# glwagner/OldOceananigans.jl

Hardware: AMD Instinct MI355X
Metric: cell_updates_per_s (higher is better)
Workload: dtype f64

## Files before the change

### oldoceananigans.jl_amd/csrc/ocn_advect_split.h

```cpp
#pragma once
#include "ocn_kernels.h"
#include "ocn_tendency_roles.h"

__global__ void __launch_bounds__(256) sum_parent_kernel(const double *__restrict__ a, const double *__restrict__ b, double *__restrict__ out, long n) {
    const long stride = (long)gridDim.x * blockDim.x;
    for (long q = (long)blockIdx.x * blockDim.x + threadIdx.x; q < n; q += stride) out[q] = a[q] + b[q];
}

template <int F, bool ACC>
__global__ void __launch_bounds__(256) advective_tendency_kernel(DGrid g, FView ua, FView va, FView wa, FView psi, FView G, Range6 r) {
    const int i = r.i0 + blockIdx.x * blockDim.x + threadIdx.x;
    const int j = r.j0 + blockIdx.y * blockDim.y + threadIdx.y;
    const int k = r.k0 + blockIdx.z;
    if (i > r.i1 || j > r.j1 || k > r.k1) return;
    double dx, dy, dz, vinv;
    if (F == F_U) {
        vinv = g.vinv_c[k - 1 + g.Hz];
        dx = mom_flux<AQ_U, 0, true, 0, true>(g, ua, psi, i, j, k) - mom_flux<AQ_U, 0, true, 0, true>(g, ua, psi, i - 1, j, k);
        dy = mom_flux<AQ_V, 0, false, 1, false>(g, va, psi, i, j + 1, k) - mom_flux<AQ_V, 0, false, 1, false>(g, va, psi, i, j, k);
        dz = mom_flux<AQ_W, 0, false, 2, false>(g, wa, psi, i, j, k + 1) - mom_flux<AQ_W, 0, false, 2, false>(g, wa, psi, i, j, k);
    } else if (F == F_V) {
        vinv = g.vinv_c[k - 1 + g.Hz];
        dx = mom_flux<AQ_U, 1, false, 0, false>(g, ua, psi, i + 1, j, k) - mom_flux<AQ_U, 1, false, 0, false>(g, ua, psi, i, j, k);
        dy = mom_flux<AQ_V, 1, true, 1, true>(g, va, psi, i, j, k) - mom_flux<AQ_V, 1, true, 1, true>(g, va, psi, i, j - 1, k);
        dz = mom_flux<AQ_W, 1, false, 2, false>(g, wa, psi, i, j, k + 1) - mom_flux<AQ_W, 1, false, 2, false>(g, wa, psi, i, j, k);
    } else if (F == F_W) {
        vinv = g.vinv_f[k - 1 + g.Hz];
        dx = mom_flux<AQ_U, 2, false, 0, false>(g, ua, psi, i + 1, j, k) - mom_flux<AQ_U, 2, false, 0, false>(g, ua, psi, i, j, k);
        dy = mom_flux<AQ_V, 2, false, 1, false>(g, va, psi, i, j + 1, k) - mom_flux<AQ_V, 2, false, 1, false>(g, va, psi, i, j, k);
        dz = mom_flux<AQ_W, 2, true, 2, true>(g, wa, psi, i, j, k) - mom_flux<AQ_W, 2, true, 2, true>(g, wa, psi, i, j, k - 1);
    } else {
        vinv = g.vinv_c[k - 1 + g.Hz];
        dx = tracer_flux<0>(g, ua, psi, i + 1, j, k) - tracer_flux<0>(g, ua, psi, i, j, k);
        dy = tracer_flux<1>(g, va, psi, i, j + 1, k) - tracer_flux<1>(g, va, psi, i, j, k);
        dz = tracer_flux<2>(g, wa, psi, i, j, k + 1) - tracer_flux<2>(g, wa, psi, i, j, k);
    }
    const double div = vinv * ((dx + dy) + dz);
    if (ACC) G.at(i, j, k) = G.at(i, j, k) - div;
    else     G.at(i, j, k) = -div + 0.0;
}

struct RoleSplitArgs : RoleArgs<OCN_MAX_FIELDS> {
    const double *A[3];
    int nrole;
    int role[OCN_MAX_FIELDS];
};

template <int TY, bool BZ, bool ACC>
__global__ void __launch_bounds__(64 * (TY + 1), OCN_ROLE_WAVES) role_split_kernel(DGrid gin, RoleSplitArgs a) {
    __shared__ double FX[2][TY][66];
    __shared__ double FY[2][TY + 1][64];

    DGrid g = gin;
    g.tx = 0; g.ty = 0; g.tz = BZ ? 1 : 0;

    const unsigned d = blockIdx.x, xcd = d & 7u, slot = d >> 3, nr = (unsigned)a.nrole;
    const unsigned pair = xcd * (unsigned)a.band + slot / nr;
    if (slot / nr >= (unsigned)a.band || pair >= (unsigned)a.npair) return;
    const int fidx = a.role[slot % nr];
    const unsigned tile = pair % (unsigned)a.ntile, chunk = pair / (unsigned)a.ntile;
    const int i0 = a.r.i0 + (int)(tile % (unsigned)a.ntile_x) * 64, j0 = a.r.j0 + (int)(tile / (unsigned)a.ntile_x) * TY;
    const int kc0 = a.r.k0 + (int)chunk * a.kchunk;
    const int kc1 = min(kc0 + a.kchunk - 1, a.r.k1);
    if (fidx == 0) role_march<ROLE_U, TY, false, BZ, 0, false, RoleSplitArgs, true, ACC>(g, a, 0, i0, j0, kc0, kc1, FX, FY);
    else if (fidx == 1) role_march<ROLE_V, TY, false, BZ, 0, false, RoleSplitArgs, true, ACC>(g, a, 1, i0, j0, kc0, kc1, FX, FY);
    else if (fidx == 2) role_march<ROLE_W, TY, false, BZ, 0, false, RoleSplitArgs, true, ACC>(g, a, 2, i0, j0, kc0, kc1, FX, FY);
    else role_march<ROLE_C, TY, false, BZ, 0, false, RoleSplitArgs, true, ACC>(g, a, fidx, i0, j0, kc0, kc1, FX, FY);
}

static inline int launch_role_split(const OcnOptions &o, const DGrid &g, hipStream_t stream, const double *const adv[3], const double *const *psi,
                                    double *const *G, const int *roles, int nrole, const int *range, bool accumulate) {
    if (nrole <= 0) return 0;
    if (nrole > OCN_MAX_FIELDS || o.arithmetic != 0) return -2;
    RoleSplitArgs a;
    for (int f = 0; f < OCN_MAX_FIELDS; ++f) { a.U[f] = nullptr; a.G[f] = nullptr; a.Un[f] = nullptr; a.Gm[f] = nullptr; a.role[f] = 0; }
    a.ftab = nullptr;
    for (int c = 0; c < 3; ++c) a.A[c] = adv[c];
    a.nrole = nrole;
    for (int q = 0; q < nrole; ++q) {
        const int f = roles[q];
        if (f < 0 || f >= OCN_MAX_FIELDS || !psi[f] || !G[f]) return -2;
        a.role[q] = f; a.U[f] = psi[f]; a.G[f] = G[f];
    }
    a.has_zeta = 0; a.store_G = 1; a.dt = 0.0; a.gamma = 0.0; a.zeta = 0.0;
    const int Px = g.Nx + 2 * g.Hx, Py = g.Ny + 2 * g.Hy;
    a.s1 = Px;
    a.s2 = (unsigned)((long)Px * Py);
    a.off = (g.Hx - 1) + (long)Px * (g.Hy - 1);
    if (range) {
        a.r = Range6{range[0], range[1], range[2], range[3], range[4], range[5]};
        a.wk0 = a.r.k0;
    } else {
        a.r = Range6{1, g.Nx, 1, g.Ny, 1, g.Nz};
        a.wk0 = (g.tz != 0 && g.Nz > 1) ? 2 : 1;
    }
    constexpr int TY = OCN_ROLE_TY;
    const int nx = a.r.i1 - a.r.i0 + 1, ny = a.r.j1 - a.r.j0 + 1, nz = a.r.k1 - a.r.k0 + 1;
    if (nx <= 0 || ny <= 0 || nz <= 0) return 0;
    a.ntile_x = (nx + 63) / 64;
    a.ntile = a.ntile_x * ((ny + TY - 1) / TY);
    a.kchunk = o.role_kchunk > 0 ? o.role_kchunk : pick_role_kchunk((long)a.ntile * nrole, nz);
    const int nchunk = (nz + a.kchunk - 1) / a.kchunk;
    a.npair = a.ntile * nchunk;
    a.band = (a.npair + 7) / 8;
    const unsigned nblocks = (unsigned)a.band * 8u * (unsigned)nrole;
    const dim3 blk(64 * (TY + 1));
#define OCN_LAUNCH_SPLIT(BZV, ACCV) hipLaunchKernelGGL((role_split_kernel<TY, BZV, ACCV>), dim3(nblocks), blk, (size_t)o.role_ldspad, stream, g, a)
    if (g.tz != 0) { if (accumulate) OCN_LAUNCH_SPLIT(true, true); else OCN_LAUNCH_SPLIT(true, false); }
    else           { if (accumulate) OCN_LAUNCH_SPLIT(false, true); else OCN_LAUNCH_SPLIT(false, false); }
#undef OCN_LAUNCH_SPLIT
    return 0;
}
```

### oldoceananigans.jl_amd/csrc/ocn_api.hip

```cpp
#include "../../include/ocn_mi355x.h"
#include "ocn_kernels.h"
#include "ocn_options.h"
#include "ocn_tendency_fused.h"
#include "ocn_tendency_roles.h"
#include "ocn_advect_split.h"
#include "ocn_epilogue_march.h"
#include "ocn_forcing.h"
#include "ocn_implicit_z.h"
#include "ocn_particles.h"
#include "ocn_open_boundary.h"
#include "ocn_diagnostics.h"
#include "ocn_boundary_function.h"
#include "ocn_forcing_function.h"
#include <hipfft/hipfft.h>
#include <array>
#include <cfloat>
#include <cmath>
#include <cstdarg>
#include <cstdio>
#include <cstdlib>
#include <cstring>
#include <memory>
#include <string>
#include <utility>
// ... 1930 lines not shown
        *slot = total ? &m->tot[f] : const_cast<double **>(&m->bg[f]);
        *loc = m->loc[f];
        return OCN_OK;
    }
    if (q[0] == 'G' || q[0] == 'M') { kind = q[0]; ++q; }
    const int f = field_index(m, q);
    if (f < 0) return fail(OCN_EINVAL, "name %s not found in model.velocities or model.tracers.", name);
    *slot = kind == 'U' ? &m->U[f] : (kind == 'G' ? &m->Gn[f] : &m->Gm[f]);
    *loc = m->loc[f];
    return OCN_OK;
}

extern "C" int ocn_model_field(ocn_model_t m, const char *name, double **ptr, int loc[3]) {
    if (!m || !name || !ptr) return fail(OCN_EINVAL, "NULL argument");
    double **slot;
    int *l;
    int rc = field_lookup(m, name, &slot, &l);
    if (rc) return rc;
    *ptr = *slot;
    if (loc) memcpy(loc, l, sizeof(int) * 3);
    return OCN_OK;
}

enum OptionScope {
    OPT_STEP,
    OPT_CREATION,
    OPT_PARTITIONED,
};
struct OptionRow {
    const char *key;
    int OcnOptions::*member;
    OptionScope scope;
    bool (*valid)(int);
    const char *range;
    const char *alias;
};
static bool nonneg(int v) { return v >= 0; }
static bool onoff(int v) { return v == 0 || v == 1; }
static constexpr int kRoleStaticLds = 8 * (2 * OCN_ROLE_TY * 66 + 2 * (OCN_ROLE_TY + 1) * 64);
static constexpr int kRoleLdspadMax = 160 * 1024 - kRoleStaticLds;
static_assert(kRoleLdspadMax == 148256 || OCN_ROLE_TY != 7, "the message of role_ldspad states the bound at TY = 7");
static bool ldspad_fits(int v) { return v >= 0 && v <= kRoleLdspadMax; }
static const OptionRow kOptions[] = {
    {"tendency_impl", &OcnOptions::tendency_impl, OPT_STEP, [](int v) { return v >= 0 && v <= 2; }, "tendency_impl is 0, 1 or 2"},
    {"arithmetic", &OcnOptions::arithmetic, OPT_STEP, [](int v) { return v == 0 || v == 1; }, "arithmetic is 0 (reference sequence) or 1 (contracted)"},
    {"role_kchunk", &OcnOptions::role_kchunk, OPT_STEP, nonneg, "role_kchunk must be >= 0 (0 = automatic)"},
    {"role_ldspad", &OcnOptions::role_ldspad, OPT_STEP, ldspad_fits, "role_ldspad is 0 .. 148256 bytes (the 160 KiB of a CU minus the kernel's own LDS)"},
    {"fused_ty", &OcnOptions::fused_ty, OPT_STEP, [](int v) { return v == 3 || v == 7; }, "fused_ty is 3 or 7"},
    {"fused_kchunk", &OcnOptions::fused_kchunk, OPT_STEP, nonneg, "fused_kchunk must be >= 0 (0 = automatic)"},
    {"fused_zwin", &OcnOptions::fused_zwin, OPT_STEP, onoff, "fused_zwin is 0 or 1"},
    {"fused_xcd", &OcnOptions::fused_xcd, OPT_STEP, onoff, "fused_xcd is 0 or 1"},
    {"epilogue_march", &OcnOptions::epilogue_march, OPT_STEP, onoff, "epilogue_march is 0 or 1"},
    {"epilogue_rows", &OcnOptions::epilogue_rows, OPT_STEP, [](int v) { return v >= 1 && v <= 8; }, "epilogue_rows is 1 .. 8"},
    {"epilogue_kchunk", &OcnOptions::epilogue_kchunk, OPT_STEP, nonneg, "epilogue_kchunk must be >= 0 (0 = automatic)"},
    {"amd_march", &OcnOptions::amd_march, OPT_STEP, onoff, "amd_march is 0 or 1"},
    {"smag_march", &OcnOptions::smag_march, OPT_STEP, onoff, "smag_march is 0 or 1"},
    {"fused_halo", &OcnOptions::fused_halo, OPT_STEP, onoff, "fused_halo is 0 or 1"},
    {"real_fft", &OcnOptions::real_fft, OPT_STEP, onoff, "real_fft is 0 or 1"},
    {"c2r_strided", &OcnOptions::c2r_strided, OPT_CREATION, onoff, "c2r_strided is 0 or 1"},
    {"fused_zfft", &OcnOptions::fused_zfft, OPT_CREATION, onoff, "fused_zfft is 0 or 1"},
    {"split_solve", &OcnOptions::split_solve, OPT_STEP, onoff, "split_solve is 0 or 1"},
    {"line_zl512", &OcnOptions::line_zl512, OPT_STEP, [](int v) { return v == 4 || v == 8; }, "line_zl512 is 4 or 8"},
    {"skip_stage_pressure", &OcnOptions::skip_stage_pressure, OPT_STEP, onoff, "skip_stage_pressure is 0 or 1"},
    {"skip_dead_tendency_store", &OcnOptions::skip_dead_tendency_store, OPT_STEP, onoff, "skip_dead_tendency_store is 0 or 1"},
    {"dist_substructured", &OcnOptions::dist_substructured, OPT_CREATION, onoff, "dist_substructured is 0 or 1"},
    {"dist_zfirst", &OcnOptions::dist_zfirst, OPT_CREATION, onoff, "dist_zfirst is 0 or 1"},
    {"dist_xfast", &OcnOptions::dist_xfast, OPT_CREATION, onoff, "dist_xfast is 0 or 1"},
    {"dist_yline", &OcnOptions::dist_yline, OPT_CREATION, onoff, "dist_yline is 0 or 1"},
    {"dist_fuse_source", &OcnOptions::dist_fuse_source, OPT_STEP, onoff, "dist_fuse_source is 0 or 1"},
    {"dist_xline_group", &OcnOptions::dist_xline_group, OPT_STEP, onoff, "dist_xline_group is 0 or 1"},
    {"dist_pencil_transposes", &OcnOptions::dist_pencil_transposes, OPT_CREATION, onoff, "dist_pencil_transposes is 0 or 1"},
    {"swap_tendencies", &OcnOptions::swap_tendencies, OPT_STEP, onoff, "swap_tendencies is 0 or 1"},
    {"fuse_substep", &OcnOptions::fuse_substep, OPT_STEP, onoff, "fuse_substep is 0 or 1"},
    {"fused_epilogue", &OcnOptions::fused_epilogue, OPT_STEP, onoff, "fused_epilogue is 0 or 1"},
    {"fused_forcing", &OcnOptions::fused_forcing, OPT_STEP, onoff, "fused_forcing is 0 or 1"},
    {"use_graph", &OcnOptions::use_graph, OPT_STEP, onoff, "use_graph is 0 or 1"},
    {"async_halos", &OcnOptions::async_halos, OPT_PARTITIONED, [](int v) { return v >= -1 && v <= 1; }, "async_halos is -1 (automatic), 0 or 1"},
    {"thin_halos", &OcnOptions::thin_halos, OPT_PARTITIONED, onoff, "thin_halos is 0 or 1"},
    {"early_exchange", &OcnOptions::early_exchange, OPT_PARTITIONED, onoff, "early_exchange is 0 or 1"},
    {"strip_width", &OcnOptions::strip_width, OPT_PARTITIONED, nonneg, "strip_width must be >= 0 (0 = automatic)"},
    {"fused_step", &OcnOptions::fused_step, OPT_PARTITIONED, onoff, "fused_step is 0 or 1", "dist_fused_step"},
};

static const OptionRow *find_option(const char *key) {
    for (const OptionRow &r : kOptions)
        if (!strcmp(key, r.key) || (r.alias && !strcmp(key, r.alias))) return &r;
    return nullptr;
}
static const OptionRow *option_row(const char *key, int value) {
    const OptionRow *r = find_option(key);
    if (!r) { fail(OCN_EINVAL, "unknown option %s", key); return nullptr; }
    if (r->valid && !r->valid(value)) { fail(OCN_EINVAL, "%s", r->range); return nullptr; }
    return r;
}

extern "C" int ocn_set_option(const char *key, int value) {
    if (!key) return fail(OCN_EINVAL, "NULL argument");
    const OptionRow *r = option_row(key, value);
    if (!r) return OCN_EINVAL;
    g_defaults.*r->member = value;
    return OCN_OK;
}

static bool dist_fused_step_buffers(const ocn_model_s *m);
static int dist_model_get_option(const ocn_model_s *m, const char *key, int *value);
static void dist_abandon_exchange(ocn_model_s *m);
extern "C" int ocn_model_set_option(ocn_model_t m, const char *key, int value) {
    if (!m || !key) return fail(OCN_EINVAL, "NULL argument");
    m->epoch += 1;
    if (!strcmp(key, "profile")) { m->profile = value; m->events_used = 0; return OCN_OK; }
    if (!strcmp(key, "forcing_function_hoist")) {
        if (value != 0 && value != 1) return fail(OCN_EINVAL, "forcing_function_hoist is 0 or 1");
        m->ff.hoist = value != 0;
        return OCN_OK;
    }
    const OptionRow *r = option_row(key, value);
    if (!r) return OCN_EINVAL;
    if (r->scope == OPT_CREATION)
        return fail(OCN_ESTATE, "option %s is read when a model is created: set it with ocn_set_option before creating the model", key);
    if (r->scope == OPT_PARTITIONED && !m->dm) return fail(OCN_EINVAL, "option %s belongs to a partitioned model", key);
    if (r->member == &OcnOptions::fused_step && value && !dist_fused_step_buffers(m))
        return fail(OCN_ENOTSUP, "fused_step needs a (connected, Periodic, Periodic) slab with the z-fastest substructured solver");
    m->opt.*r->member = value;
    return OCN_OK;
}

static int model_ivd_form(const ocn_model_s *) { return 0; }

static int count_background(const ocn_model_s *m) {
    int n = 0;
    for (int f = 0; f < m->nf; ++f) n += m->bg[f] ? 1 : 0;
    return n;
}
static bool has_background(const ocn_model_s *m) { return count_background(m) > 0; }
static bool has_background_velocity(const ocn_model_s *m) { return m->bg[0] || m->bg[1] || m->bg[2]; }
static const double *total_velocity(const ocn_model_s *m, int c) { return m->bg[c] ? m->tot[c] : m->U[c]; }
static int update_total_velocities(ocn_model_s *m) {
    for (int c = 0; c < 3; ++c)
        if (m->bg[c]) {
            int rc = sum_parent(m->grid->d, m->U[c], m->bg[c], m->loc[c], m->tot[c]);
            if (rc) return rc;
        }
    return OCN_OK;
}

static bool has_forcing(const ocn_model_s *m) {
    for (int f = 0; f < m->nf; ++f)
        if (m->forcing_h.nterms[f] > 0) return true;
    return false;
}
static int evaluate_boundary_functions(ocn_model_s *m) {
    if (m->bf.n == 0) return OCN_OK;
    BfFields fields = {};
    for (int f = 0; f < m->nf; ++f) fields.p[f] = m->U[f];
    int na = 1, nb = 1;
    for (int q = 0; q < m->bf.n; ++q) { na = std::max(na, m->bf.slot[q].fn.Na); nb = std::max(nb, m->bf.slot[q].fn.Nb); }
    bf_launch(m->bf.table_d, m->bf.n, na, nb, fields, m->time);
    KERNEL_CHECK();
    return OCN_OK;
}

static int count_linear_flux(const ocn_model_s *m) {
    int n = 0;
    for (int f = 0; f < m->nf; ++f)
        for (int sd = 0; sd < 6; ++sd) n += m->lin[f][sd].on ? 1 : 0;
    return n;
}

struct StepPlan {
// ... 1565 lines not shown
```

### oldoceananigans.jl_amd/csrc/ocn_options.h

```cpp
#pragma once

struct OcnOptions {
    int tendency_impl = 2;
    int arithmetic = 0;
    int role_kchunk = 0;
    int role_ldspad = 0;
    int fused_ty = 7;
    int fused_kchunk = 0;
    int fused_zwin = 1;
    int fused_xcd = 0;
    int epilogue_march = 1;
    int epilogue_rows = 4;
    int epilogue_kchunk = 0;
    int amd_march = 1;
    int smag_march = 1;
    int fused_halo = 1;
    int real_fft = 1;
    int c2r_strided = 1;
    int fused_zfft = 1;
    int split_solve = 1;
    int line_zl512 = 4;
    int skip_stage_pressure = 1;
    int skip_dead_tendency_store = 1;
    int dist_substructured = 1;
    int dist_zfirst = 1;
    int dist_xfast = 1;
    int dist_yline = 1;
    int dist_fuse_source = 1;
    int dist_xline_group = 1;
    int dist_pencil_transposes = 1;
    int swap_tendencies = 1;
    int fuse_substep = 1;
    int fused_epilogue = 1;
    int fused_forcing = 1;
    int use_graph = 0;
    int async_halos = -1;
    int thin_halos = 1;
    int early_exchange = 1;
    int strip_width = 0;
    int fused_step = 1;
};
```

### oldoceananigans.jl_amd/csrc/ocn_tendency_roles.h

```cpp
#pragma once
#include "ocn_tendency_fused.h"
#include "ocn_forcing.h"

#ifndef OCN_ROLE_WAVES
#define OCN_ROLE_WAVES 6
#endif
#ifndef OCN_ROLE_TY
#define OCN_ROLE_TY 7
#endif
#ifndef OCN_ROLE_PF
#define OCN_ROLE_PF 1
#endif
#ifndef OCN_ROLE_ABLATE
#define OCN_ROLE_ABLATE 0
#endif
#ifndef OCN_ROLE_STORE_AUX
#define OCN_ROLE_STORE_AUX 2
#endif
#ifndef OCN_ROLE_GM_AUX
#define OCN_ROLE_GM_AUX 0
#endif
enum { ROLE_U = 0, ROLE_V = 1, ROLE_W = 2, ROLE_C = 3 };

template <int NF>
struct RoleArgs {
    const double *U[NF];
    double *G[NF];
    double *Un[NF];
    const double *Gm[NF];
    int s1;
    unsigned s2;
    long off;
    Range6 r;
    int wk0;
    int kchunk, ntile_x, ntile, npair, band;
    int has_zeta;
    int store_G;
    double dt, gamma, zeta;
    const ForcingTable *ftab;
};

typedef __amdgpu_buffer_rsrc_t Rsrc;
typedef unsigned v2u __attribute__((ext_vector_type(2)));
typedef const double __attribute__((address_space(4))) *KTab;
__device__ __forceinline__ KTab ktab(const double *p) { return (KTab)p; }
#define ROLE_OOB 0x80000000u
__device__ __forceinline__ Rsrc make_rsrc(const void *p) {
    return __builtin_amdgcn_make_buffer_rsrc(const_cast<void *>(p), 0, (int)ROLE_OOB, 0x00020000);
}
template <int IMM> __device__ __forceinline__ double ldb(Rsrc r, unsigned voff, unsigned soff) {
    return __builtin_bit_cast(double, __builtin_amdgcn_raw_buffer_load_b64(r, (int)(voff + (unsigned)IMM), (int)soff, 0));
}
template <int IMM> __device__ __forceinline__ double ldb_once(Rsrc r, unsigned voff, unsigned soff) {
    return __builtin_bit_cast(double, __builtin_amdgcn_raw_buffer_load_b64(r, (int)(voff + (unsigned)IMM), (int)soff, OCN_ROLE_GM_AUX));
}
template <int IMM> __device__ __forceinline__ void stb(Rsrc r, unsigned voff, unsigned soff, double v) {
    __builtin_amdgcn_raw_buffer_store_b64(__builtin_bit_cast(v2u, v), r, (int)(voff + (unsigned)IMM), (int)soff, OCN_ROLE_STORE_AUX);
}

struct ColOff { unsigned c; unsigned s1; };

template <bool OWN> __device__ __forceinline__ Win6 xwin6(Rsrc b, unsigned so, const ColOff &o, double centre) {
    Win6 w;
    w.s[0] = ldb<0>(b, o.c, so); w.s[1] = ldb<8>(b, o.c, so); w.s[2] = ldb<16>(b, o.c, so);
    w.s[3] = OWN ? centre : ldb<24>(b, o.c, so);
    w.s[4] = ldb<32>(b, o.c, so); w.s[5] = ldb<40>(b, o.c, so);
    return w;
}
__device__ __forceinline__ Win6 xwin4(Rsrc b, unsigned so, const ColOff &o) {
    Win6 w;
    w.s[0] = 0.0; w.s[5] = 0.0;
    w.s[1] = ldb<8>(b, o.c, so); w.s[2] = ldb<16>(b, o.c, so); w.s[3] = ldb<24>(b, o.c, so); w.s[4] = ldb<32>(b, o.c, so);
    return w;
}
template <bool OWN> __device__ __forceinline__ Win6 ywin6(Rsrc b, unsigned so, const ColOff &o, double centre) {
    Win6 w;
#pragma unroll
    for (int n = 0; n < 6; ++n) w.s[n] = (OWN && n == 3) ? centre : ldb<24>(b, o.c, so + (unsigned)(n - 3) * o.s1);
    return w;
}
__device__ __forceinline__ Win6 ywin4(Rsrc b, unsigned so, const ColOff &o) {
    Win6 w;
    w.s[0] = 0.0; w.s[5] = 0.0;
#pragma unroll
    for (int n = 1; n < 5; ++n) w.s[n] = ldb<24>(b, o.c, so + (unsigned)(n - 3) * o.s1);
    return w;
}
__device__ __forceinline__ Win6 zwin4(Rsrc b, unsigned so, const ColOff &o, unsigned s2) {
    Win6 w;
    w.s[0] = 0.0; w.s[5] = 0.0;
    w.s[1] = ldb<24>(b, o.c, so - 2u * s2); w.s[2] = ldb<24>(b, o.c, so - s2); w.s[3] = ldb<24>(b, o.c, so); w.s[4] = ldb<24>(b, o.c, so + s2);
    return w;
}

struct PlaneCtx {
    Rsrc u, v, w, q;
    unsigned so;
    unsigned s2;
    double axk, ayk;
    const double *axz, *ayz;
};

template <int ROLE, bool SPLIT = false> __device__ __forceinline__ Win6 load_zin(const PlaneCtx &p, unsigned so, const ColOff &o) {
    if (SPLIT && ROLE == ROLE_W) return zwin4(p.w, so, o, p.s2);
    if (ROLE == ROLE_U) return xwin4(p.w, so, o);
    if (ROLE == ROLE_V) return ywin4(p.w, so, o);
    Win6 w;
#pragma unroll
    for (int n = 0; n < 6; ++n) w.s[n] = 0.0;
    if (ROLE == ROLE_C) w.s[3] = ldb<24>(p.w, o.c, so);
    return w;
}
template <int ROLE, int ARITH, bool SPLIT = false>
__device__ __forceinline__ double z_flux(const DGrid &g, const Win6 &zin, int i, int j, int k, const Win6 &qz) {
    const bool bx = g.tx != 0, by = g.ty != 0, bz = g.tz != 0;
    const double az = g.az;
    if (ROLE == ROLE_U) {
        const double wt = sym4<ARITH>(zin, az, bx, i, false, g.Nx);
// ... 163 lines not shown
        if (OCN_ROLE_PF == 2) vmov(qn, qnn);
        if (SUB || ACC) vmov(gm, gmn);
        if ((SUB || ACC) && OCN_ROLE_PF == 2) vmov(gmn, gmnn);
        zin = load_zin<ROLE, SPLIT>(p, p.so, o);
    };
    auto z_compute = [&](const DGrid &gg, const int k, const int buf, const long pk) {
        const double fz = z_flux<ROLE, ARITH, SPLIT>(gg, zin, i, j, k, qz);
        const int pb = buf ^ 1;
        const long pkm = pk - 1;
        const double vinv = ROLE == ROLE_W ? ktab(g.vinv_f)[pkm] : ktab(g.vinv_c)[pkm];
        const double dx = FX[pb][row0][lane + 1] - FX[pb][row0][lane];
        const double dy = FY[pb][row0 + 1][lane] - FY[pb][row0][lane];
        const double div = vinv * ((dx + dy) + (fz - fz_prev));
        Gn = ACC ? gm - div : -div + 0.0;
        if (FORCE) {
            if (a.ftab->nterms[fidx] > 0)
                Gn = Gn + forcing_sum(a.ftab, fidx, g, min(i, a.r.i1), min(j, a.r.j1), max(k - 1, a.r.k0), qz.s[2]);
        }
        store = cell_r && k > kc0 && (ROLE != ROLE_W || k - 1 >= a.wk0) && (!(OCN_ROLE_ABLATE & 4) || Gn == 1.2345);
        if (SUB) {
            Uv = qz.s[2];
            if (a.has_zeta) Uv += a.dt * (a.gamma * Gn + a.zeta * gm);
            else            Uv += a.dt * a.gamma * Gn;
        }
        fz_prev = fz;
    };
    auto stores = [&]() {
        const unsigned st = o.c | (store ? 0u : ROLE_OOB);
        stb<24>(rG, st | g_oob, (OCN_ROLE_ABLATE & 64) ? s2 * 3u : p.so - s2, Gn);
        if (SUB) stb<24>(rUn, st, (OCN_ROLE_ABLATE & 64) ? s2 * 3u : p.so - s2, Uv);
    };

    for (int k = kc0; k <= kc1; ++k) {
        const int buf = k & 1;
        const long pk = (long)(k - 1 + Hz);
        p.axk = ktab(g.ax)[pk]; p.ayk = ktab(g.ay)[pk];
        p.axz = g.ax + pk - 2; p.ayz = g.ay + pk - 2;
        asm volatile("" : "+v"(o.c));
        z_loads();
        Win6 qx, xaux, qy, yaux;
        auto x_loads = [&]() {
            qx = (OCN_ROLE_ABLATE & 8) ? qz : xwin6<true>(p.q, p.so, o, qz.s[3]);
            xaux = ROLE == ROLE_W ? zwin4(p.u, p.so, o, s2) : load_xaux<ROLE, SPLIT>(p, o);
        };
        auto y_loads = [&]() {
            qy = (OCN_ROLE_ABLATE & 8) ? qz : ywin6<true>(p.q, p.so, o, qz.s[3]);
            yaux = ROLE == ROLE_W ? zwin4(p.v, p.so, o, s2) : load_yaux<ROLE, SPLIT>(p, o);
        };
        auto prefetches = [&]() {
            if (OCN_ROLE_PF == 2) {
                qnn = ldb<24>(p.q, o.c, (OCN_ROLE_ABLATE & 1) ? p.so : p.so + (k < kc1 ? 4u : 3u) * s2);
                if ((SUB || ACC) && !(OCN_ROLE_ABLATE & 2)) gmnn = ldb_once<24>(rGm, o.c | cell_off, p.so + s2);
                return;
            }
            qn = ldb<24>(p.q, o.c, (OCN_ROLE_ABLATE & 1) ? p.so : p.so + 3u * s2);
            if ((SUB || ACC) && !(OCN_ROLE_ABLATE & 2)) gmn = ldb_once<24>(rGm, o.c | cell_off, p.so);
        };
        auto plane = [&](const DGrid &gg) {
            __builtin_amdgcn_sched_barrier(0);
            z_compute(gg, k, buf, pk);
            __builtin_amdgcn_sched_barrier(0);
            x_loads();
            stores();
            __builtin_amdgcn_sched_barrier(0);
            FX[buf][row0][lane] = x_flux<ROLE, ARITH, SPLIT>(gg, p, qx, xaux, i, j, k);
            __builtin_amdgcn_sched_barrier(0);
            y_loads();
            prefetches();
            __builtin_amdgcn_sched_barrier(0);
            FY[buf][row0][lane] = y_flux<ROLE, ARITH, SPLIT>(gg, p, qy, yaux, i, j, k);
        };
        if (near_wall(k)) plane(gB); else plane(gP);
        p.so += s2;
        role_barrier();
    }
    {
        const int k = kc1 + 1;
        z_loads();
        if (near_wall(k)) z_compute(gB, k, k & 1, (long)(k - 1 + Hz)); else z_compute(gP, k, k & 1, (long)(k - 1 + Hz));
        stores();
    }
}

template <int NTR, int TY, bool BZ, bool SUB, int ARITH = 0, bool FORCE = false>
__global__ void __launch_bounds__(64 * (TY + 1), OCN_ROLE_WAVES) role_tendency_kernel(DGrid gin, RoleArgs<3 + NTR> a) {
    constexpr int NF = 3 + NTR;
    __shared__ double FX[2][TY][66];
    __shared__ double FY[2][TY + 1][64];

    DGrid g = gin;
    g.tx = 0; g.ty = 0; g.tz = BZ ? 1 : 0;

    const unsigned d = blockIdx.x, xcd = d & 7u, slot = d >> 3;
    const unsigned role = slot % NF, pair = xcd * (unsigned)a.band + slot / NF;
    if (slot / NF >= (unsigned)a.band || pair >= (unsigned)a.npair) return;
    const unsigned tile = pair % (unsigned)a.ntile, chunk = pair / (unsigned)a.ntile;
    const int i0 = a.r.i0 + (int)(tile % (unsigned)a.ntile_x) * 64, j0 = a.r.j0 + (int)(tile / (unsigned)a.ntile_x) * TY;
    const int kc0 = a.r.k0 + (int)chunk * a.kchunk;
    const int kc1 = min(kc0 + a.kchunk - 1, a.r.k1);
    if (role == 0) role_march<ROLE_U, TY, SUB, BZ, ARITH, FORCE>(g, a, 0, i0, j0, kc0, kc1, FX, FY);
    else if (role == 1) role_march<ROLE_V, TY, SUB, BZ, ARITH, FORCE>(g, a, 1, i0, j0, kc0, kc1, FX, FY);
    else if (role == 2) role_march<ROLE_W, TY, SUB, BZ, ARITH, FORCE>(g, a, 2, i0, j0, kc0, kc1, FX, FY);
    else role_march<ROLE_C, TY, SUB, BZ, ARITH, FORCE>(g, a, (int)role, i0, j0, kc0, kc1, FX, FY);
}

static inline bool role_tendency_supported(const OcnOptions &o, const DGrid &g) {
    const double plane = 8.0 * (g.Nx + 2.0 * g.Hx) * (g.Ny + 2.0 * g.Hy);
    return plane * ((o.role_kchunk > 0 ? o.role_kchunk : 64) + 8.0) < 2147483648.0;
}

static inline int pick_role_kchunk(long tiles_roles, int nz) {
    int best = nz;
    double best_cost = -1;
    const long slots = (long)((4 * OCN_ROLE_WAVES) / (OCN_ROLE_TY + 1)) * g_num_cus;
    for (int kc = 8; kc <= 64; ++kc) {
        if (kc > nz && kc != 8) break;
        const int nchunk = (nz + kc - 1) / kc;
        const int kce = (nz + nchunk - 1) / nchunk;
        const long blocks = tiles_roles * nchunk;
        const double per_block = kce + 1.5;
        const double cost = (double)blocks * per_block / slots + per_block;
        if (best_cost < 0 || cost < best_cost) { best_cost = cost; best = kce; }
    }
    return best;
}

template <int NTR, int TY>
static int launch_roles_t(const OcnOptions &o, const DGrid &g, hipStream_t stream, RoleArgs<3 + NTR> &a, bool sub) {
    constexpr int NF = 3 + NTR;
    const int nx = a.r.i1 - a.r.i0 + 1, ny = a.r.j1 - a.r.j0 + 1, nz = a.r.k1 - a.r.k0 + 1;
    if (nx <= 0 || ny <= 0 || nz <= 0) return 0;
    a.ntile_x = (nx + 63) / 64;
    a.ntile = a.ntile_x * ((ny + TY - 1) / TY);
    a.kchunk = o.role_kchunk > 0 ? o.role_kchunk : pick_role_kchunk((long)a.ntile * NF, nz);
    const int nchunk = (nz + a.kchunk - 1) / a.kchunk;
    a.npair = a.ntile * nchunk;
    a.band = (a.npair + 7) / 8;
    const unsigned nblocks = (unsigned)a.band * 8u * NF;
    const dim3 blk(64 * (TY + 1));
#define OCN_LAUNCH_ROLES(BZV, SUBV, AR) hipLaunchKernelGGL((role_tendency_kernel<NTR, TY, BZV, SUBV, AR>), dim3(nblocks), blk, (size_t)o.role_ldspad, stream, g, a)
#define OCN_LAUNCH_ROLES_F(BZV, SUBV) hipLaunchKernelGGL((role_tendency_kernel<NTR, TY, BZV, SUBV, 0, true>), dim3(nblocks), blk, (size_t)o.role_ldspad, stream, g, a)
    if (a.ftab) {
        if (o.arithmetic != 0 || g.tz != 0) return -2;
        if (sub) OCN_LAUNCH_ROLES_F(false, true); else OCN_LAUNCH_ROLES_F(false, false);
    } else if (o.arithmetic == 1) {
        if (g.tz != 0) { if (sub) OCN_LAUNCH_ROLES(true, true, 1); else OCN_LAUNCH_ROLES(true, false, 1); }
        else           { if (sub) OCN_LAUNCH_ROLES(false, true, 1); else OCN_LAUNCH_ROLES(false, false, 1); }
    } else {
        if (g.tz != 0) { if (sub) OCN_LAUNCH_ROLES(true, true, 0); else OCN_LAUNCH_ROLES(true, false, 0); }
        else           { if (sub) OCN_LAUNCH_ROLES(false, true, 0); else OCN_LAUNCH_ROLES(false, false, 0); }
    }
#undef OCN_LAUNCH_ROLES_F
#undef OCN_LAUNCH_ROLES
    return 0;
}

template <int NTR>
static int launch_roles_n(const OcnOptions &o, const DGrid &g, hipStream_t stream, const double *u, const double *v, const double *w, const double *const *tr,
                          double *Gu, double *Gv, double *Gw, double *const *Gc, const int *range, const FusedSubstep *sub,
                          const ForcingTable *ftab) {
    constexpr int NF = 3 + NTR;
    RoleArgs<NF> a;
    a.ftab = ftab;
    a.U[0] = u; a.U[1] = v; a.U[2] = w; a.G[0] = Gu; a.G[1] = Gv; a.G[2] = Gw;
    for (int t = 0; t < NTR; ++t) { a.U[3 + t] = tr[t]; a.G[3 + t] = Gc[t]; }
    a.has_zeta = sub ? sub->has_zeta : 0;
    a.store_G = (sub && !sub->store_G) ? 0 : 1;
    a.dt = sub ? sub->dt : 0.0; a.gamma = sub ? sub->gamma : 0.0; a.zeta = sub ? sub->zeta : 0.0;
    for (int f = 0; f < NF; ++f) { a.Un[f] = sub ? sub->Un[f] : nullptr; a.Gm[f] = sub ? sub->Gm[f] : nullptr; }
    const int Px = g.Nx + 2 * g.Hx, Py = g.Ny + 2 * g.Hy;
    a.s1 = Px;
    a.s2 = (unsigned)((long)Px * Py);
    a.off = (g.Hx - 1) + (long)Px * (g.Hy - 1);
    if (range) {
        a.r = Range6{range[0], range[1], range[2], range[3], range[4], range[5]};
        a.wk0 = a.r.k0;
    } else {
        a.r = Range6{1, g.Nx, 1, g.Ny, 1, g.Nz};
        a.wk0 = (g.tz != 0 && g.Nz > 1) ? 2 : 1;
    }
    return launch_roles_t<NTR, OCN_ROLE_TY>(o, g, stream, a, sub != nullptr);
}

static inline int launch_role_tendency(const OcnOptions &o, const DGrid &g, hipStream_t stream, const double *u, const double *v, const double *w,
                                       const double *const *tr, int ntr, double *Gu, double *Gv, double *Gw, double *const *Gc,
                                       const int *range, const FusedSubstep *sub = nullptr, const ForcingTable *ftab = nullptr) {
    switch (ntr) {
        case 0: return launch_roles_n<0>(o, g, stream, u, v, w, tr, Gu, Gv, Gw, Gc, range, sub, ftab);
        case 1: return launch_roles_n<1>(o, g, stream, u, v, w, tr, Gu, Gv, Gw, Gc, range, sub, ftab);
        case 2: return launch_roles_n<2>(o, g, stream, u, v, w, tr, Gu, Gv, Gw, Gc, range, sub, ftab);
        case 3: return launch_roles_n<3>(o, g, stream, u, v, w, tr, Gu, Gv, Gw, Gc, range, sub, ftab);
        default: return -2;
    }
}
```

Before: 2.794 billion.

## Schedule role kernels with graded vertical chunks balanced across XCDs

Replaces the uniform k-chunk split of the role tendency and advection-split kernels with a precomputed schedule of chunk-length classes (long chunks first, short ones last), dealt across the 8 XCDs to balance work and shrink the tail wave. The schedule is built on the host, cached, and passed in the kernel argument struct, and each block locates its tile and k-range by walking the class table. This costs extra per-block index arithmetic, a larger kernel argument, and more halo reloads from short chunks, and it is on by default via a new role_schedule option.

```diff
diff --git a/oldoceananigans.jl_amd/csrc/ocn_advect_split.h b/oldoceananigans.jl_amd/csrc/ocn_advect_split.h
--- a/oldoceananigans.jl_amd/csrc/ocn_advect_split.h
+++ b/oldoceananigans.jl_amd/csrc/ocn_advect_split.h
@@ -54,14 +54,10 @@
     DGrid g = gin;
     g.tx = 0; g.ty = 0; g.tz = BZ ? 1 : 0;
 
-    const unsigned d = blockIdx.x, xcd = d & 7u, slot = d >> 3, nr = (unsigned)a.nrole;
-    const unsigned pair = xcd * (unsigned)a.band + slot / nr;
-    if (slot / nr >= (unsigned)a.band || pair >= (unsigned)a.npair) return;
-    const int fidx = a.role[slot % nr];
-    const unsigned tile = pair % (unsigned)a.ntile, chunk = pair / (unsigned)a.ntile;
-    const int i0 = a.r.i0 + (int)(tile % (unsigned)a.ntile_x) * 64, j0 = a.r.j0 + (int)(tile / (unsigned)a.ntile_x) * TY;
-    const int kc0 = a.r.k0 + (int)chunk * a.kchunk;
-    const int kc1 = min(kc0 + a.kchunk - 1, a.r.k1);
+    unsigned q;
+    int i0, j0, kc0, kc1;
+    if (!role_block<TY>(a, (unsigned)a.nrole, q, i0, j0, kc0, kc1)) return;
+    const int fidx = a.role[q];
     if (fidx == 0) role_march<ROLE_U, TY, false, BZ, 0, false, RoleSplitArgs, true, ACC>(g, a, 0, i0, j0, kc0, kc1, FX, FY);
     else if (fidx == 1) role_march<ROLE_V, TY, false, BZ, 0, false, RoleSplitArgs, true, ACC>(g, a, 1, i0, j0, kc0, kc1, FX, FY);
     else if (fidx == 2) role_march<ROLE_W, TY, false, BZ, 0, false, RoleSplitArgs, true, ACC>(g, a, 2, i0, j0, kc0, kc1, FX, FY);
@@ -95,15 +91,8 @@
         a.wk0 = (g.tz != 0 && g.Nz > 1) ? 2 : 1;
     }
     constexpr int TY = OCN_ROLE_TY;
-    const int nx = a.r.i1 - a.r.i0 + 1, ny = a.r.j1 - a.r.j0 + 1, nz = a.r.k1 - a.r.k0 + 1;
-    if (nx <= 0 || ny <= 0 || nz <= 0) return 0;
-    a.ntile_x = (nx + 63) / 64;
-    a.ntile = a.ntile_x * ((ny + TY - 1) / TY);
-    a.kchunk = o.role_kchunk > 0 ? o.role_kchunk : pick_role_kchunk((long)a.ntile * nrole, nz);
-    const int nchunk = (nz + a.kchunk - 1) / a.kchunk;
-    a.npair = a.ntile * nchunk;
-    a.band = (a.npair + 7) / 8;
-    const unsigned nblocks = (unsigned)a.band * 8u * (unsigned)nrole;
+    const unsigned nblocks = role_launch_geometry<TY>(o, g, a, nrole);
+    if (nblocks == 0) return 0;
     const dim3 blk(64 * (TY + 1));
 #define OCN_LAUNCH_SPLIT(BZV, ACCV) hipLaunchKernelGGL((role_split_kernel<TY, BZV, ACCV>), dim3(nblocks), blk, (size_t)o.role_ldspad, stream, g, a)
     if (g.tz != 0) { if (accumulate) OCN_LAUNCH_SPLIT(true, true); else OCN_LAUNCH_SPLIT(true, false); }
diff --git a/oldoceananigans.jl_amd/csrc/ocn_api.hip b/oldoceananigans.jl_amd/csrc/ocn_api.hip
--- a/oldoceananigans.jl_amd/csrc/ocn_api.hip
+++ b/oldoceananigans.jl_amd/csrc/ocn_api.hip
@@ -2036,9 +2036,16 @@
     {"fused_step", &OcnOptions::fused_step, OPT_PARTITIONED, onoff, "fused_step is 0 or 1", "dist_fused_step"},
 };
 
+static const OptionRow kLaunchKeys[] = {
+    {"role_schedule", &OcnOptions::role_schedule, OPT_STEP, onoff, "role_schedule is 0 (one uniform chunk length) or 1 (graded chunks)"},
+    {"role_slots", &OcnOptions::role_slots, OPT_STEP, nonneg, "role_slots must be >= 0 (0 = the device's resident workgroups)"},
+};
+
 static const OptionRow *find_option(const char *key) {
     for (const OptionRow &r : kOptions)
         if (!strcmp(key, r.key) || (r.alias && !strcmp(key, r.alias))) return &r;
+    for (const OptionRow &r : kLaunchKeys)
+        if (!strcmp(key, r.key)) return &r;
     return nullptr;
 }
 static const OptionRow *option_row(const char *key, int value) {
diff --git a/oldoceananigans.jl_amd/csrc/ocn_options.h b/oldoceananigans.jl_amd/csrc/ocn_options.h
--- a/oldoceananigans.jl_amd/csrc/ocn_options.h
+++ b/oldoceananigans.jl_amd/csrc/ocn_options.h
@@ -5,6 +5,8 @@
     int arithmetic = 0;
     int role_kchunk = 0;
     int role_ldspad = 0;
+    int role_schedule = 1;
+    int role_slots = 0;
     int fused_ty = 7;
     int fused_kchunk = 0;
     int fused_zwin = 1;
diff --git a/oldoceananigans.jl_amd/csrc/ocn_role_schedule.h b/oldoceananigans.jl_amd/csrc/ocn_role_schedule.h
--- /dev/null
+++ b/oldoceananigans.jl_amd/csrc/ocn_role_schedule.h
@@ -0,0 +1,194 @@
+#pragma once
+
+#if defined(__HIPCC__) || defined(__CUDACC__)
+#define OCN_HD __host__ __device__ __forceinline__
+#else
+#define OCN_HD inline
+#endif
+
+enum { ROLE_NXCD = 8, ROLE_MAX_CLASS = 16, ROLE_SHORTEST = 8, ROLE_LONGEST = 24, ROLE_LONGEST_DEEP = 64 };
+static const double ROLE_CHUNK_COST = 0.6;
+static const double ROLE_TAIL_FRACTION = 0.1;
+static const double ROLE_ROUND_SPREAD = 1.08;
+static const double ROLE_LADDER_GROWTH = 1.25;
+
+struct RoleClass {
+    int k0;
+    int len;
+    int nchunk;
+};
+
+struct RoleSchedule {
+    int nclass;
+    int band;
+    RoleClass cls[ROLE_MAX_CLASS];
+    int cnt[ROLE_MAX_CLASS][ROLE_NXCD];
+};
+
+OCN_HD bool role_schedule_locate(const RoleSchedule &s, unsigned xcd, unsigned pairslot, unsigned ntile, unsigned *tile, int *k0, int *len) {
+    unsigned before = 0;
+    for (int c = 0; c < s.nclass; ++c) {
+        const unsigned n = (unsigned)s.cnt[c][xcd];
+        if (pairslot < before + n) {
+            unsigned q = pairslot - before;
+            for (unsigned x = 0; x < xcd; ++x) q += (unsigned)s.cnt[c][x];
+            *tile = q % ntile;
+            *k0 = s.cls[c].k0 + (int)(q / ntile) * s.cls[c].len;
+            *len = s.cls[c].len;
+            return true;
+        }
+        before += n;
+    }
+    return false;
+}
+
+static inline int role_schedule_max_len(double plane_bytes) {
+    const double planes = 2147483648.0 / plane_bytes;
+    if (planes <= 9.0) return 0;
+    if (planes > 1e9) return 1000000000;
+    int n = (int)planes;
+    if ((double)n * plane_bytes >= 2147483648.0) --n;
+    return n - 8;
+}
+
+static inline int role_schedule_chunks(const RoleSchedule &s) {
+    int n = 0;
+    for (int c = 0; c < s.nclass; ++c) n += s.cls[c].nchunk;
+    return n;
+}
+
+static inline double role_schedule_cost(const RoleSchedule &s, long ncol_pairs, int nroles, long slots) {
+    if (s.nclass == 0) return 0.0;
+    double column = 0.0;
+    for (int c = 0; c < s.nclass; ++c) column += (double)s.cls[c].nchunk * (s.cls[c].len + ROLE_CHUNK_COST);
+    const double longest = ROLE_ROUND_SPREAD * (s.cls[0].len + ROLE_CHUNK_COST), last = s.cls[s.nclass - 1].len + ROLE_CHUNK_COST;
+    const double blocks = (double)ncol_pairs * nroles * role_schedule_chunks(s);
+    if (blocks <= (double)slots) return longest;
+    const double cost = (double)ncol_pairs * nroles * column / (double)slots + ROLE_TAIL_FRACTION * last;
+    return cost > longest ? cost : longest;
+}
+
+static inline double role_schedule_imbalance(const RoleSchedule &s, double *work = nullptr) {
+    double w[ROLE_NXCD], mean = 0.0, worst = 0.0;
+    for (int x = 0; x < ROLE_NXCD; ++x) {
+        w[x] = 0.0;
+        for (int c = 0; c < s.nclass; ++c) w[x] += (double)s.cnt[c][x] * s.cls[c].len;
+        mean += w[x] / ROLE_NXCD;
+        if (work) work[x] = w[x];
+    }
+    for (int x = 0; x < ROLE_NXCD; ++x) { const double d = w[x] > mean ? w[x] - mean : mean - w[x]; if (d > worst) worst = d; }
+    return worst;
+}
+
+static inline bool role_schedule_push(RoleSchedule &s, int len, int n) {
+    if (n <= 0) return true;
+    if (s.nclass > 0 && s.cls[s.nclass - 1].len == len) { s.cls[s.nclass - 1].nchunk += n; return true; }
+    if (s.nclass == ROLE_MAX_CLASS) return false;
+    s.cls[s.nclass].k0 = 0; s.cls[s.nclass].len = len; s.cls[s.nclass].nchunk = n;
+    ++s.nclass;
+    return true;
+}
+
+static inline void role_schedule_deal(RoleSchedule &s, long ncol_pairs) {
+    for (int i = 1; i < s.nclass; ++i)
+        for (int j = i; j > 0 && s.cls[j].len > s.cls[j - 1].len; --j) { const RoleClass t = s.cls[j]; s.cls[j] = s.cls[j - 1]; s.cls[j - 1] = t; }
+    int nc = 0;
+    for (int c = 0; c < s.nclass; ++c) {
+        if (nc > 0 && s.cls[nc - 1].len == s.cls[c].len) s.cls[nc - 1].nchunk += s.cls[c].nchunk;
+        else s.cls[nc++] = s.cls[c];
+    }
+    s.nclass = nc;
+    int k = 0;
+    for (int c = 0; c < s.nclass; ++c) { s.cls[c].k0 = k; k += s.cls[c].len * s.cls[c].nchunk; }
+    long work[ROLE_NXCD] = {0};
+    for (int c = 0; c < s.nclass; ++c) {
+        const long pairs = ncol_pairs * s.cls[c].nchunk, len = s.cls[c].len;
+        long lo = work[0], hi = work[0];
+        for (int x = 1; x < ROLE_NXCD; ++x) { if (work[x] < lo) lo = work[x]; if (work[x] > hi) hi = work[x]; }
+        long loose = ((hi - lo) / len + 2) * ROLE_NXCD;
+        if (loose > pairs) loose = pairs;
+        loose += (pairs - loose) % ROLE_NXCD;
+        const long base = (pairs - loose) / ROLE_NXCD;
+        for (int x = 0; x < ROLE_NXCD; ++x) { s.cnt[c][x] = (int)base; work[x] += base * len; }
+        for (long p = 0; p < loose; ++p) {
+            int best = 0;
+            for (int x = 1; x < ROLE_NXCD; ++x) if (work[x] < work[best]) best = x;
+            s.cnt[c][best] += 1; work[best] += len;
+        }
+    }
+    s.band = 0;
+    for (int x = 0; x < ROLE_NXCD; ++x) {
+        int n = 0;
+        for (int c = 0; c < s.nclass; ++c) n += s.cnt[c][x];
+        if (n > s.band) s.band = n;
+    }
+}
+
+static inline RoleSchedule role_schedule_uniform(long ncol_pairs, int nz, int nchunk) {
+    RoleSchedule s = {};
+    const int q = nz / nchunk, r = nz % nchunk;
+    role_schedule_push(s, q + 1, r);
+    role_schedule_push(s, q, nchunk - r);
+    role_schedule_deal(s, ncol_pairs);
+    return s;
+}
+
+static inline RoleSchedule role_schedule_graded(long ncol_pairs, int nz, double ratio, int max_len) {
+    RoleSchedule s = {};
+    const int longest = ratio >= 2.0 ? ROLE_LONGEST_DEEP : ROLE_LONGEST;
+    if (max_len > longest) max_len = longest;
+    int left = nz, after = 0, want = ROLE_SHORTEST, last = 0;
+    for (;;) {
+        const double allowed = ROLE_LADDER_GROWTH * ratio * after;
+        want = ROLE_SHORTEST;
+        while (2 * want <= allowed && 2 * want <= max_len) want *= 2;
+        if (allowed >= max_len || want > max_len) want = max_len;
+        if (left < want + ROLE_SHORTEST) break;
+        if (!role_schedule_push(s, want, 1)) { s.nclass = 0; return s; }
+        left -= want; after += want; last = want;
+    }
+    if (left > 0) {
+        if (left < ROLE_SHORTEST && last > 0) {
+            RoleClass &top = s.cls[s.nclass - 1];
+            left += top.len;
+            if (--top.nchunk == 0) --s.nclass;
+        }
+        const int nhead = (left + max_len - 1) / max_len, q = left / nhead, r = left % nhead;
+        if (s.nclass + 2 > ROLE_MAX_CLASS) { s.nclass = 0; return s; }
+        role_schedule_push(s, q + 1, r);
+        role_schedule_push(s, q, nhead - r);
+    }
+    role_schedule_deal(s, ncol_pairs);
+    return s;
+}
+
+static inline bool role_schedule_balanced(const RoleSchedule &s) {
+    return s.nclass > 0 && role_schedule_imbalance(s) <= (double)s.cls[s.nclass - 1].len;
+}
+
+static inline RoleSchedule role_schedule_build(long ncol_pairs, int nz, long slots, int nxcd, int max_len, int nroles = 1) {
+    RoleSchedule best = {};
+    if (ncol_pairs <= 0 || nz <= 0 || nxcd != ROLE_NXCD || max_len < 1) return best;
+    if (slots < 1) slots = 1;
+    const int nmin = (nz + max_len - 1) / max_len;
+    best = role_schedule_uniform(ncol_pairs, nz, nmin);
+    double best_cost = role_schedule_cost(best, ncol_pairs, nroles, slots);
+    bool best_ok = role_schedule_balanced(best);
+    auto consider = [&](const RoleSchedule &s) {
+        if (s.nclass == 0 || s.cls[0].len > max_len) return;
+        const bool ok = role_schedule_balanced(s);
+        const double cost = role_schedule_cost(s, ncol_pairs, nroles, slots);
+        if ((ok && !best_ok) || (ok == best_ok && cost < best_cost)) { best = s; best_cost = cost; best_ok = ok; }
+    };
+    const int nshort = nz / ROLE_SHORTEST;
+    if (nshort > nmin) consider(role_schedule_uniform(ncol_pairs, nz, nshort));
+    if (nz >= 2 * ROLE_SHORTEST && max_len >= ROLE_SHORTEST) {
+        double ratio = (double)ncol_pairs * nroles / (double)slots;
+        for (int step = 0; step < 8; ++step, ratio *= 0.5) consider(role_schedule_graded(ncol_pairs, nz, ratio, max_len));
+    }
+    if (!best_ok) {
+        for (int len = nz < max_len ? nz : max_len; len >= 1; --len)
+            if (nz % len == 0) { const RoleSchedule s = role_schedule_uniform(ncol_pairs, nz, nz / len); if (role_schedule_balanced(s)) { best = s; break; } }
+    }
+    return best;
+}
diff --git a/oldoceananigans.jl_amd/csrc/ocn_tendency_roles.h b/oldoceananigans.jl_amd/csrc/ocn_tendency_roles.h
--- a/oldoceananigans.jl_amd/csrc/ocn_tendency_roles.h
+++ b/oldoceananigans.jl_amd/csrc/ocn_tendency_roles.h
@@ -1,6 +1,7 @@
 #pragma once
 #include "ocn_tendency_fused.h"
 #include "ocn_forcing.h"
+#include "ocn_role_schedule.h"
 
 #ifndef OCN_ROLE_WAVES
 #define OCN_ROLE_WAVES 6
@@ -34,6 +35,7 @@
     Range6 r;
     int wk0;
     int kchunk, ntile_x, ntile, npair, band;
+    RoleSchedule sched;
     int has_zeta;
     int store_G;
     double dt, gamma, zeta;
@@ -363,6 +365,28 @@
     }
 }
 
+template <int TY, class Args>
+__device__ __forceinline__ bool role_block(const Args &a, unsigned nf, unsigned &role, int &i0, int &j0, int &kc0, int &kc1) {
+    const unsigned d = blockIdx.x, xcd = d & 7u, slot = d >> 3, pairslot = slot / nf;
+    role = slot % nf;
+    unsigned tile;
+    if (a.sched.nclass > 0) {
+        int k0, len;
+        if (!role_schedule_locate(a.sched, xcd, pairslot, (unsigned)a.ntile, &tile, &k0, &len)) return false;
+        kc0 = a.r.k0 + k0;
+        kc1 = kc0 + len - 1;
+    } else {
+        const unsigned pair = xcd * (unsigned)a.band + pairslot;
+        if (pairslot >= (unsigned)a.band || pair >= (unsigned)a.npair) return false;
+        tile = pair % (unsigned)a.ntile;
+        kc0 = a.r.k0 + (int)(pair / (unsigned)a.ntile) * a.kchunk;
+        kc1 = min(kc0 + a.kchunk - 1, a.r.k1);
+    }
+    i0 = a.r.i0 + (int)(tile % (unsigned)a.ntile_x) * 64;
+    j0 = a.r.j0 + (int)(tile / (unsigned)a.ntile_x) * TY;
+    return true;
+}
+
 template <int NTR, int TY, bool BZ, bool SUB, int ARITH = 0, bool FORCE = false>
 __global__ void __launch_bounds__(64 * (TY + 1), OCN_ROLE_WAVES) role_tendency_kernel(DGrid gin, RoleArgs<3 + NTR> a) {
     constexpr int NF = 3 + NTR;
@@ -372,22 +396,20 @@
     DGrid g = gin;
     g.tx = 0; g.ty = 0; g.tz = BZ ? 1 : 0;
 
-    const unsigned d = blockIdx.x, xcd = d & 7u, slot = d >> 3;
-    const unsigned role = slot % NF, pair = xcd * (unsigned)a.band + slot / NF;
-    if (slot / NF >= (unsigned)a.band || pair >= (unsigned)a.npair) return;
-    const unsigned tile = pair % (unsigned)a.ntile, chunk = pair / (unsigned)a.ntile;
-    const int i0 = a.r.i0 + (int)(tile % (unsigned)a.ntile_x) * 64, j0 = a.r.j0 + (int)(tile / (unsigned)a.ntile_x) * TY;
-    const int kc0 = a.r.k0 + (int)chunk * a.kchunk;
-    const int kc1 = min(kc0 + a.kchunk - 1, a.r.k1);
+    unsigned role;
+    int i0, j0, kc0, kc1;
+    if (!role_block<TY>(a, NF, role, i0, j0, kc0, kc1)) return;
     if (role == 0) role_march<ROLE_U, TY, SUB, BZ, ARITH, FORCE>(g, a, 0, i0, j0, kc0, kc1, FX, FY);
     else if (role == 1) role_march<ROLE_V, TY, SUB, BZ, ARITH, FORCE>(g, a, 1, i0, j0, kc0, kc1, FX, FY);
     else if (role == 2) role_march<ROLE_W, TY, SUB, BZ, ARITH, FORCE>(g, a, 2, i0, j0, kc0, kc1, FX, FY);
     else role_march<ROLE_C, TY, SUB, BZ, ARITH, FORCE>(g, a, (int)role, i0, j0, kc0, kc1, FX, FY);
 }
 
+static inline int role_max_len(const DGrid &g) { return role_schedule_max_len(8.0 * (g.Nx + 2.0 * g.Hx) * (g.Ny + 2.0 * g.Hy)); }
 static inline bool role_tendency_supported(const OcnOptions &o, const DGrid &g) {
-    const double plane = 8.0 * (g.Nx + 2.0 * g.Hx) * (g.Ny + 2.0 * g.Hy);
-    return plane * ((o.role_kchunk > 0 ? o.role_kchunk : 64) + 8.0) < 2147483648.0;
+    const int max_len = role_max_len(g);
+    if (o.role_kchunk > 0) return o.role_kchunk <= max_len;
+    return max_len >= (o.role_schedule ? (int)ROLE_SHORTEST : 64);
 }
 
 static inline int pick_role_kchunk(long tiles_roles, int nz) {
@@ -406,18 +428,56 @@
     return best;
 }
 
-template <int NTR, int TY>
-static int launch_roles_t(const OcnOptions &o, const DGrid &g, hipStream_t stream, RoleArgs<3 + NTR> &a, bool sub) {
-    constexpr int NF = 3 + NTR;
+static inline const RoleSchedule &role_schedule_for(long ntile, int nz, long slots, int max_len, int nroles) {
+    struct Entry { long ntile, slots; int nz, max_len, nroles; RoleSchedule s; };
+    thread_local Entry cache[4] = {};
+    thread_local int next = 0;
+    for (Entry &e : cache)
+        if (e.ntile == ntile && e.nz == nz && e.slots == slots && e.max_len == max_len && e.nroles == nroles) return e.s;
+    Entry &e = cache[next];
+    next = (next + 1) % 4;
+    e.ntile = ntile; e.nz = nz; e.slots = slots; e.max_len = max_len; e.nroles = nroles;
+    e.s = role_schedule_build(ntile, nz, slots, ROLE_NXCD, max_len, nroles);
+    return e.s;
+}
+
+template <int TY, class Args>
+static unsigned role_launch_geometry(const OcnOptions &o, const DGrid &g, Args &a, int nroles) {
     const int nx = a.r.i1 - a.r.i0 + 1, ny = a.r.j1 - a.r.j0 + 1, nz = a.r.k1 - a.r.k0 + 1;
     if (nx <= 0 || ny <= 0 || nz <= 0) return 0;
     a.ntile_x = (nx + 63) / 64;
     a.ntile = a.ntile_x * ((ny + TY - 1) / TY);
-    a.kchunk = o.role_kchunk > 0 ? o.role_kchunk : pick_role_kchunk((long)a.ntile * NF, nz);
-    const int nchunk = (nz + a.kchunk - 1) / a.kchunk;
-    a.npair = a.ntile * nchunk;
-    a.band = (a.npair + 7) / 8;
-    const unsigned nblocks = (unsigned)a.band * 8u * NF;
+    a.sched = RoleSchedule{};
+    if (o.role_kchunk == 0 && o.role_schedule) {
+        const long slots = o.role_slots > 0 ? o.role_slots : (long)((4 * OCN_ROLE_WAVES) / (OCN_ROLE_TY + 1)) * g_num_cus;
+        a.sched = role_schedule_for(a.ntile, nz, slots, role_max_len(g), nroles);
+#ifdef OCN_ROLE_LADDER_ENV
+        if (const char *env = getenv("OCN_ROLE_LADDER")) {
+            RoleSchedule s = {};
+            int sum = 0;
+            for (const char *p = env; *p;) { const int len = atoi(p); if (len <= 0 || len > role_max_len(g) || !role_schedule_push(s, len, 1)) { sum = -1; break; } sum += len; while (*p && *p != ',') ++p; if (*p) ++p; }
+            if (sum == nz) { role_schedule_deal(s, a.ntile); a.sched = s; }
+        }
+#endif
+    }
+    if (a.sched.nclass > 0) {
+        a.kchunk = a.sched.cls[0].len;
+        a.npair = a.ntile * role_schedule_chunks(a.sched);
+        a.band = a.sched.band;
+    } else {
+        a.kchunk = o.role_kchunk > 0 ? o.role_kchunk : pick_role_kchunk((long)a.ntile * nroles, nz);
+        const int nchunk = (nz + a.kchunk - 1) / a.kchunk;
+        a.npair = a.ntile * nchunk;
+        a.band = (a.npair + 7) / 8;
+    }
+    return (unsigned)a.band * 8u * (unsigned)nroles;
+}
+
+template <int NTR, int TY>
+static int launch_roles_t(const OcnOptions &o, const DGrid &g, hipStream_t stream, RoleArgs<3 + NTR> &a, bool sub) {
+    constexpr int NF = 3 + NTR;
+    const unsigned nblocks = role_launch_geometry<TY>(o, g, a, NF);
+    if (nblocks == 0) return 0;
     const dim3 blk(64 * (TY + 1));
 #define OCN_LAUNCH_ROLES(BZV, SUBV, AR) hipLaunchKernelGGL((role_tendency_kernel<NTR, TY, BZV, SUBV, AR>), dim3(nblocks), blk, (size_t)o.role_ldspad, stream, g, a)
 #define OCN_LAUNCH_ROLES_F(BZV, SUBV) hipLaunchKernelGGL((role_tendency_kernel<NTR, TY, BZV, SUBV, 0, true>), dim3(nblocks), blk, (size_t)o.role_ldspad, stream, g, a)
```

Measured after the change: 2.796 billion, median of 6. Within noise of the previous version (+0.1%).
